# idra-lab/safe-mpc

Measured on AMD Instinct MI355X. Metric: RTI-MPC instance-steps/s (batch=4096 per GPU, Z1 N=30), higher is better.
Workload: dtype f64; 1 GPU; C1: Z1-class 6-DoF, N=30, 4096 instances/GPU, controller st (soft terminal NN row, MLP 12-256-256-256-1 fp32), EXT cost exact Hessian, 6 capsule pairs, Halton x0; batch_per_gpu=4096, batch_total=4096, horizon=30, controller=st, streams_per_gpu=3, qp_form=throughput, hip_graphs=False

## Files before the change

### safe_mpc_amd/csrc/engine.hip

```cpp
#include <hip/hip_runtime.h>

#include <cstdarg>
#include <cstdio>
#include <cstring>
#include <new>
#include <type_traits>
#include <vector>

#include "../../include/smpc.h"
#include "kernel_qp.hpp"
#include "kernel_qp_wg.hpp"
#include "kernel_build.hpp"
#include "kernels_callers.hpp"
#include "kernels_policy.hpp"
#include "kernels_mlp.hpp"
#include "kernels_nodes.hpp"
#include "kernels_sqp.hpp"
#include "kernels_guess.hpp"
#include "kernels_score.hpp"
#include "kernels_ik.hpp"
#include "kernels_rays.hpp"
#include "kernels_forecast.hpp"

using namespace smpc;
// ... 83 lines not shown
    DevBuf<double> d_nn;
    DevBuf<double> d_ws;
    int qp_mode = -2;
    DevBuf<double> d_hrec;
    bool wg_lds_raised[2] = {false, false};
    DevBuf<int32_t> d_order, d_last_it;
    int order_B = 0;
    DevBuf<int32_t> d_ord_hist;
    DevBuf<float> d_S, d_y, d_GS, d_dA, d_dB;
    DevBuf<int32_t> d_nn_idx;
    int32_t* d_nn_cnt = nullptr;
    DevBuf<float> d_act[SMPC_MAX_LAYERS];
    DevBuf<float> d_dg[SMPC_MAX_LAYERS];
    DevBuf<char> d_stage;
    ParamBlock chk{"check bounds"};
    ParamBlock gchk{"guess check bounds"};
    ParamBlock schk{"score bounds"};
    ParamBlock ikb{"inverse kinematics bounds"};
    DevBuf<char> d_roll;
    int timing = 0;
    int timed = 0;
    static constexpr int EV_RING = 64;
    hipEvent_t ev_sets[EV_RING][5] = {};
    bool ev_complete[EV_RING] = {};
    hipEvent_t* ev_t = ev_sets[0];
    int ev_cur = 0;
    bool timing_now = false;
    long timed_count = 0;
    std::vector<smpc_handle*> kids;
    hipEvent_t ev_fork = nullptr, ev_join = nullptr;
    DevBuf<unsigned long long> d_wstat;
    const uint8_t* d_active = nullptr;
    DevBuf<char> d_polw;
    float last_ms[4] = {0, 0, 0, 0};
    long mlp_rows_whole = 0;
    long mlp_rows_hint = 0;
    DevBuf<char> d_par;
    DevBuf<char> d_sqp;
    DevBuf<int32_t> d_guess;
    DevBuf<char> d_score;
    char err[256] = "";
};

namespace {

int fail(smpc_handle* h, int code, const char* fmt, ...) {
    char* dst = h ? h->err : g_create_err;
    va_list ap;
    va_start(ap, fmt);
    vsnprintf(dst, 256, fmt, ap);
    va_end(ap);
    return code;
}
#define HIPCHK(h, expr)                                                                                       \
    do {                                                                                                      \
        hipError_t e_ = (expr);                                                                               \
        if (e_ != hipSuccess) return fail(h, SMPC_EHIP, "%s failed: %s", #expr, hipGetErrorString(e_));        \
    } while (0)

bool capturing(const smpc_handle* h) {
    hipStreamCaptureStatus cs = hipStreamCaptureStatusNone;
    if (hipStreamIsCapturing(h->stream, &cs) != hipSuccess) { (void)hipGetLastError(); return false; }
    return cs != hipStreamCaptureStatusNone;
}

}
// ... 143 lines not shown
    HIPCHK(h, hipMemcpyAsync(h->d_lo.p, l.data(), l.size() * sizeof(double), hipMemcpyHostToDevice, h->stream));
    HIPCHK(h, hipMemcpyAsync(h->d_hi.p, u.data(), u.size() * sizeof(double), hipMemcpyHostToDevice, h->stream));
    HIPCHK(h, hipStreamSynchronize(h->stream));
    return SMPC_OK;
}

int ensure_mlp(smpc_handle* h, size_t M, int level = 2) {
    const size_t Mp = (M + 127) / 128 * 128, row = sizeof(float) * Mp, H = h->net->H;
    int rc;
    if ((rc = h->d_y.reserve(h, "network output", row))) return rc;
    for (int l = 0; level >= 1 && l + 1 < h->net->nlayers; l++)
        if ((rc = h->d_dg[l].reserve(h, "network activation derivatives", row * H))) return rc;
    if (level < 2) return SMPC_OK;
    if ((rc = h->d_S.reserve(h, "network features", row * MLP_KPAD)) || (rc = h->d_GS.reserve(h, "network gradients", row * MLP_NPAD)) ||
        (rc = h->d_dA.reserve(h, "network backward pass", row * H)) || (rc = h->d_dB.reserve(h, "network backward pass", row * H)))
        return rc;
    for (int l = 0; l + 1 < h->net->nlayers; l++)
        if ((rc = h->d_act[l].reserve(h, "network activations", row * H))) return rc;
    return SMPC_OK;
}

int ensure_nn_idx(smpc_handle* h, size_t M) {
    if (sizeof(int32_t) * (M + 1) <= h->d_nn_idx.cap) return SMPC_OK;
    const int rc = h->d_nn_idx.reserve(h, "network row list", sizeof(int32_t) * (M + 1));
    h->d_nn_cnt = h->d_nn_idx.cap ? h->d_nn_idx.p + h->d_nn_idx.cap / sizeof(int32_t) - 1 : nullptr;
    if (rc) return rc;
    HIPCHK(h, hipMemsetAsync(h->d_nn_cnt, 0, sizeof(int32_t), h->stream));
    return SMPC_OK;
}

CtxSrc rows_of_nodes(int per) { CtxSrc c; c.per = per; return c; }
CtxSrc rows_step_major(int B, long m0) { CtxSrc c; c.mod = B; c.m0 = (int)(m0 % B); c.j0 = (int)(m0 / B); return c; }

template <int NQ> int run_mlp(smpc_handle* h, int M, int mode, int N, const double* d_x, bool backward, CtxSrc rows,
                              const double* d_p = nullptr, double* d_ev = nullptr, bool* chained = nullptr, int compact = 0) {
    int rc;
    const Net& net = *h->net;
    CtxSrc cx = rows;
    if (net.n_ctx > 0) {
        const float* own = h->ctx.held();
        cx.n = net.n_ctx;
        cx.p = own ? own : net.d_default_ctx.p;
        cx.stride = own ? net.n_ctx : 0;
        cx.T = own ? (int)h->ctx_T : 1;
        cx.clock = cx.T > 1 && cx.mod == 0 && !(own && h->ctx_fc) ? h->scene_clock : nullptr;
    }
    const int Mp = (M + 127) / 128 * 128, H = net.H, L = net.nlayers;
    hipStream_t s = h->stream;
    const int32_t* idx = mode == 3 ? h->d_nn_idx.p : nullptr;
    const int32_t* live = mode == 3 ? h->d_nn_cnt : nullptr;
    if (chained) *chained = false;
    {
        const long rows_all = h->mlp_rows_whole > 0 ? (h->mlp_rows_whole + 127) / 128 * 128
                                                    : (h->mlp_rows_hint > 0 && mode == 3 ? (h->mlp_rows_hint + 127) / 128 * 128 : (long)Mp);
        static const bool no_fused = getenv("SMPC_MLP_UNFUSED") != nullptr;
        static const long fused_max = [] { const char* e = getenv("SMPC_MLP_FUSED_MAX"); return e ? atol(e) : 8192L; }();
        if (!no_fused && rows_all < fused_max && H == MLPF_H && L == 4 && (!backward || (d_p && d_ev))) {
            if ((rc = ensure_mlp(h, (size_t)M, 0))) return rc;
            MlpWeights Wt;
            for (int l = 0; l < SMPC_MAX_LAYERS; l++) { Wt.wf[l] = net.Wfwd[l]; Wt.wb[l] = net.Wbwd[l]; Wt.bias[l] = net.bias[l]; }
            const dim3 grd((M + MLPF_ROWS - 1) / MLPF_ROWS), blk(256);
            if (backward)
                hipLaunchKernelGGL((k_mlp_fused<NQ, true>), grd, blk, 0, s, h->d_desc, M, N, mode, net.act, Wt, d_x, d_p, idx, live, h->d_y.p, d_ev,
                                   compact, cx);
            else
                hipLaunchKernelGGL((k_mlp_fused<NQ, false>), grd, blk, 0, s, h->d_desc, M, N, mode, net.act, Wt, d_x, d_p, idx, live, h->d_y.p,
                                   (double*)nullptr, 0, cx);
            HIPCHK(h, hipGetLastError());
            if (chained) *chained = backward;
            return SMPC_OK;
        }
        static const bool large_chain = [] { const char* e = getenv("SMPC_MLP_LARGE"); return e && !strcmp(e, "chain"); }();
        if (!no_fused && !large_chain && rows_all >= fused_max && H == MLPF_H && L == 4 && (!backward || (d_p && d_ev))) {
            if ((rc = ensure_mlp(h, (size_t)M, backward ? 1 : 0))) return rc;
            MlpWeights Wt;
            for (int l = 0; l < SMPC_MAX_LAYERS; l++) { Wt.wf[l] = net.Wfwd[l]; Wt.wb[l] = net.Wbwd[l]; Wt.bias[l] = net.bias[l]; }
            const dim3 grd((M + MLPF_ROWS - 1) / MLPF_ROWS), blk(64);
            if (backward)
                hipLaunchKernelGGL((k_mlp_wave<NQ, true>), grd, blk, 0, s, h->d_desc, M, N, mode, net.act, Wt, d_x, d_p, idx, live, h->d_y.p, d_ev,
                                   compact, h->d_dg[0].p, h->d_dg[1].p, h->d_dg[2].p, cx);
            else
                hipLaunchKernelGGL((k_mlp_wave<NQ, false>), grd, blk, 0, s, h->d_desc, M, N, mode, net.act, Wt, d_x, d_p, idx, live, h->d_y.p,
                                   (double*)nullptr, 0, (float*)nullptr, (float*)nullptr, (float*)nullptr, cx);
            HIPCHK(h, hipGetLastError());
            if (chained) *chained = backward;
            return SMPC_OK;
        }
    }
    if ((rc = ensure_mlp(h, (size_t)M))) return rc;
    hipLaunchKernelGGL((k_nn_features<NQ>), dim3((Mp + 63) / 64), dim3(64), 0, s, h->d_desc, M, Mp, N, mode, d_x,
                       h->d_S.p, idx, live, cx);
    const dim3 blk(64), grd(Mp / 32, H / 64);
    hipLaunchKernelGGL((k_gemm_f32<EPI_BIAS_GELU>), grd, blk, 0, s, Mp, H, MLP_KPAD, h->d_S.p, net.Wfwd[0], net.bias[0],
                       (const float*)nullptr, h->d_act[0].p, h->d_dg[0].p, live, net.act);
    for (int l = 1; l + 1 < L; l++)
        hipLaunchKernelGGL((k_gemm_f32<EPI_BIAS_GELU>), grd, blk, 0, s, Mp, H, H, h->d_act[l - 1].p, net.Wfwd[l], net.bias[l],
                           (const float*)nullptr, h->d_act[l].p, h->d_dg[l].p, live, net.act);
    hipLaunchKernelGGL(k_nn_output, dim3((Mp + 3) / 4), dim3(256), 0, s, Mp, H, h->d_act[L - 2].p, h->d_dg[L - 2].p,
                       net.Wbwd[L - 1], net.bias[L - 1], h->d_y.p, h->d_dA.p, live);
    if (backward) {
        float *cur = h->d_dA.p, *nxt = h->d_dB.p;
        for (int l = L - 2; l >= 1; l--) {
            hipLaunchKernelGGL((k_gemm_f32<EPI_MUL>), grd, blk, 0, s, Mp, H, H, cur, net.Wbwd[l], (const float*)nullptr,
                               h->d_dg[l - 1].p, nxt, (float*)nullptr, live, net.act);
            float* t = cur; cur = nxt; nxt = t;
        }
        hipLaunchKernelGGL((k_gemm_f32<EPI_PLAIN>), dim3(Mp / 32, MLP_NPAD / 64), blk, 0, s, Mp, MLP_NPAD, H, cur,
                           net.Wbwd[0], (const float*)nullptr, (const float*)nullptr, h->d_GS.p, (float*)nullptr, live, net.act);
    }
    HIPCHK(h, hipGetLastError());
    return SMPC_OK;
}

template <int NQ>
int launch_nn(smpc_handle* h, int B, const double* d_xg, const double* d_p, double* d_out, int compact) {
    if (h->desc.nn_mode == SMPC_NN_NONE) return SMPC_OK;
    const int N = h->N;
    hipStream_t s = h->stream;
    if (h->net->nlayers == 0) return fail(h, SMPC_ESTATE, "nn_mode != NONE but smpc_set_mlp was not called");
    const int mode = h->desc.nn_mode == SMPC_NN_TERMINAL ? 1 : 3;
    const int M = mode == 1 ? B : B * N;
    int rc;
    if (mode == 3) {
        if ((rc = ensure_nn_idx(h, (size_t)M))) return rc;
        hipLaunchKernelGGL(k_nn_compact, dim3((M + 63) / 64), dim3(64), 0, s, M, N, d_p, h->d_nn_idx.p, h->d_nn_cnt);
    }
    bool chained = false;
    if ((rc = run_mlp<NQ>(h, M, mode, N, d_xg, true, rows_of_nodes(N + 1), d_p, d_out, &chained, compact))) return rc;
    if (!chained)
        hipLaunchKernelGGL((k_nn_chain<NQ>), dim3((M + 63) / 64), dim3(64), 0, s, h->d_desc, M, N, mode, d_xg, d_p,
                           h->d_y.p, h->d_GS.p, d_out, mode == 3 ? h->d_nn_idx.p : (const int32_t*)nullptr,
                           mode == 3 ? h->d_nn_cnt : (const int32_t*)nullptr, compact);
    HIPCHK(h, hipGetLastError());
    return SMPC_OK;
}

template <class F> int with_scene(const smpc_handle* h, int B, F&& f, int64_t off = 0, bool clocked = true) {
    if (const double* geom = h->scene.for_batch(B)) {
        if (h->scene_fc) return f(std::true_type{}, SceneSrc{geom, nullptr, h->scene_T, 0});
        return f(std::true_type{}, SceneSrc{geom, clocked && h->scene_T > 1 ? h->scene_clock : nullptr, h->scene_T, off});
    }
    return f(std::false_type{}, (const double*)nullptr);
}

template <class F> int with_model(const smpc_handle* h, int B, F&& f) {
    if (const ModelSrc table = h->models.for_batch(B)) return f(std::true_type{}, table);
    return f(std::false_type{});
}

int guard_scene_and_context(smpc_handle* h, int B, const char* who) {
    const int rc = h->scene.guard(h, B, who);
    return rc ? rc : h->ctx.guard(h, B, who);
}
int guard_scene_context_and_models(smpc_handle* h, int B, const char* who) {
    const int rc = guard_scene_and_context(h, B, who);
    return rc ? rc : h->models.guard(h, B, who);
}

void drop_forecast(smpc_handle* h) {
    if (h->scene_fc) h->scene.clear();
    if (h->ctx_fc) h->ctx.clear();
// ... 764 lines not shown

extern "C" {

int smpc_abi_version(void) { return SMPC_ABI_VERSION; }

const char* smpc_last_error(const smpc_handle* h) { return h ? h->err : g_create_err; }

int smpc_create(const smpc_problem_desc* desc, int device, smpc_handle** out) {
    if (!desc || !out) return fail(nullptr, SMPC_EINVAL, "null argument");
    *out = nullptr;
    if (stream_route() < 0)
        return fail(nullptr, SMPC_EINVAL, "SMPC_STREAM_PRIORITY=%s: expected default, high or low", getenv("SMPC_STREAM_PRIORITY"));
    if (desc->abi_version != SMPC_ABI_VERSION)
        return fail(nullptr, SMPC_EINVAL, "descriptor ABI %d, library ABI %d", desc->abi_version, SMPC_ABI_VERSION);
    if (desc->nq < 5 || desc->nq > SMPC_MAX_NQ) return fail(nullptr, SMPC_EINVAL, "nq=%d unsupported", desc->nq);
    if (desc->N < 1 || desc->N > SMPC_MAX_N) return fail(nullptr, SMPC_EINVAL, "N=%d outside 1..%d", desc->N, SMPC_MAX_N);
    if (desc->n_rows < 0 || desc->n_rows > SMPC_MAX_ROWS || desc->n_points < 1 || desc->n_points > SMPC_MAX_POINTS)
        return fail(nullptr, SMPC_EINVAL, "n_rows / n_points out of range");
    for (int i = 0; i < desc->n_points; i++)
        if (desc->points[i].link >= desc->nq) return fail(nullptr, SMPC_EINVAL, "point %d rides on link %d >= nq", i, desc->points[i].link);
    for (int r = 0; r < desc->n_rows; r++) {
        const smpc_row& row = desc->rows[r];
        if (row.kind < 0 || row.kind > SMPC_ROW_COORD || row.pa < 0 || row.pa >= desc->n_points)
            return fail(nullptr, SMPC_EINVAL, "row %d malformed", r);
    }
    if (3 * desc->nq + desc->n_rows + 1 > 32)
        return fail(nullptr, SMPC_EINVAL, "3*nq + n_rows + 1 = %d constraint rows per stage exceed the 32 lanes of a half-wavefront",
                    3 * desc->nq + desc->n_rows + 1);
    int ndev = 0;
    if (hipGetDeviceCount(&ndev) != hipSuccess || ndev <= 0)
        return fail(nullptr, SMPC_EHIP, "no HIP device visible: the engine has no CPU fallback");
    if (device < 0 || device >= ndev) return fail(nullptr, SMPC_EINVAL, "device %d of %d", device, ndev);
    smpc_handle* h = new (std::nothrow) smpc_handle();
    if (!h) return fail(nullptr, SMPC_ENOMEM, "out of host memory");
    h->desc = *desc;
    h->device = device;
    h->N = desc->N;
    hipError_t e = create_handle_stream(device, &h->stream);
    if (e == hipSuccess) e = hipMalloc((void**)&h->d_desc, sizeof(smpc_problem_desc));
    if (e == hipSuccess) e = hipMemcpy(h->d_desc, desc, sizeof(smpc_problem_desc), hipMemcpyHostToDevice);
    for (int i = 0; i < 5 * smpc_handle::EV_RING && e == hipSuccess; i++) e = hipEventCreate(&h->ev_sets[i / 5][i % 5]);
    if (e != hipSuccess) {
        fail(nullptr, SMPC_EHIP, "device setup failed: %s", hipGetErrorString(e));
        smpc_destroy(h);
        return SMPC_EHIP;
    }
    int rc = upload_bounds(h, nullptr, nullptr);
    if (rc) {
        snprintf(g_create_err, sizeof(g_create_err), "%s", h->err);
        smpc_destroy(h);
        return rc;
    }
    *out = h;
    return SMPC_OK;
}

void smpc_destroy(smpc_handle* h) {
    if (!h) return;
    (void)hipSetDevice(h->device);
    for (smpc_handle* k : h->kids) smpc_destroy(k);
    if (h->stream) (void)hipStreamSynchronize(h->stream);
    if (h->ev_fork) (void)hipEventDestroy(h->ev_fork);
    if (h->ev_join) (void)hipEventDestroy(h->ev_join);
    for (auto& set : h->ev_sets) for (auto& e : set) if (e) (void)hipEventDestroy(e);
    if (h->stream) (void)hipStreamDestroy(h->stream);
    if (h->d_desc) (void)hipFree(h->d_desc);
// ... 697 lines not shown
    if (B <= 0 || !par || !st || !x || !u_out || !abort_out || !any_abort) return fail(h, SMPC_EINVAL, "bad argument");
    if (!st->x_guess || !st->u_guess || !st->x_temp || !st->u_temp || !st->p || !st->x_viable || !st->fails ||
        !st->current_step || !st->status || !st->qp_iter)
        return fail(h, SMPC_EINVAL, "policy state incomplete");
    const int kind = par->kind;
    if (kind < SMPC_POLICY_NAIVE || kind > SMPC_POLICY_PARALLEL) return fail(h, SMPC_EINVAL, "unknown policy kind %d", kind);
    const bool receding = kind == SMPC_POLICY_RECEDING || kind == SMPC_POLICY_REAL_RECEDING;
    const bool parallel = kind == SMPC_POLICY_PARALLEL;
    if ((receding || parallel) && !st->r) return fail(h, SMPC_EINVAL, "receding policy without r");
    if (parallel && h->desc.nn_mode != SMPC_NN_ALL) return fail(h, SMPC_EINVAL, "parallel policy needs the safe-set row on every node (SMPC_NN_ALL)");
    if (kind == SMPC_POLICY_REAL_RECEDING && (!par->stage_lo || !par->stage_hi)) return fail(h, SMPC_EINVAL, "stage_lo / stage_hi missing");
    if (stepping && !u_other) return fail(h, SMPC_EINVAL, "u_other missing");
    if (kind != SMPC_POLICY_NAIVE && (!par->x_min || !par->x_max || (h->desc.n_rows > 0 && (!par->row_lb_chk || !par->row_ub_chk))))
        return fail(h, SMPC_EINVAL, "check bounds missing");
    if ((receding || parallel) && h->net->nlayers == 0) return fail(h, SMPC_ESTATE, "receding policy but smpc_set_mlp was not called");
    if (parallel)
        if (const int rf = refuse_slots(h, "smpc_policy_step", "the parallel policy's candidate slots are not instances",
                                            {&h->scene, &h->ctx, &h->models}))
            return rf;
    (void)hipSetDevice(h->device);
    const int N = h->N, nq = h->desc.nq, nx = 2 * nq;
    hipStream_t s = h->stream;
    int rc;
    if ((rc = guard_scene_context_and_models(h, B, "smpc_policy_step"))) return rc;
    TrajSrc tr;
    if (!parallel && (rc = policy_traj_src(h, B, st, &tr))) return rc;
    if ((rc = ensure_batch(h, B))) return rc;
    PolScratch w;
    if ((rc = policy_scratch(h, B, &w))) return rc;
    int32_t *d_ok = w.ok, *d_safe = w.safe, *d_acc = w.acc;
    uint8_t* d_act = w.act;
    if (kind != SMPC_POLICY_NAIVE && (rc = upload_check_bounds(h, par->x_min, par->x_max, par->row_lb_chk, par->row_ub_chk))) return rc;
    if (parallel) return policy_step_parallel(h, B, par, st, x, stepping, u_other, u_out, abort_out, any_abort, d_ok, d_safe, d_acc, d_act);
    if (kind != SMPC_POLICY_REAL_RECEDING)
        hipLaunchKernelGGL(k_guess_correction, dim3((B * nq + 63) / 64), dim3(64), 0, s, B, N, nq, h->desc.dt, st->x_guess,
                           st->u_guess, stepping, any_abort, d_ok);
    if (receding) {
        if (kind == SMPC_POLICY_REAL_RECEDING) {
            if ((rc = ensure_instance_bounds(h, B, true))) return rc;
            h->bounds.commit(B);
        }
        hipLaunchKernelGGL(k_policy_pre, dim3((unsigned)(((size_t)B * (N + 1) + 63) / 64)), dim3(64), 0, s, B, N, nx, kind,
                           stepping, st->r, st->p, st->x_guess, par->stage_lo, par->stage_hi, par->tube, h->bounds.d.p, instance_hi(h),
                           kind == SMPC_POLICY_REAL_RECEDING ? any_abort : (int32_t*)nullptr,
                           kind == SMPC_POLICY_REAL_RECEDING ? d_ok : (int32_t*)nullptr);
    }
    if (tr.p)
        hipLaunchKernelGGL(k_policy_traj, dim3((unsigned)(((size_t)B * (N + 1) + 63) / 64)), dim3(64), 0, s, B, N, stepping,
                           st->current_step, tr.p, tr.len, tr.stride, st->p);
    HIPCHK(h, hipGetLastError());
    h->d_active = stepping;
    h->mlp_rows_hint = receding ? 2L * B : 0L;
    rc = with_nq(h, [&](auto NQ) { return launch_solve<NQ>(h, B, x, st->x_guess, st->u_guess, st->p, st->x_temp, st->u_temp, st->status, st->qp_iter); });
    h->d_active = nullptr;
    if (rc) { h->mlp_rows_hint = 0; return rc; }
    if (kind != SMPC_POLICY_NAIVE) {
        const int coll = par->collision_first_node ? 1 : N + 1;
        if (receding) {
            const size_t M = (size_t)B * (N + 1);
            if ((rc = ensure_nn_idx(h, M))) return rc;
            hipLaunchKernelGGL(k_policy_safe_list, dim3((unsigned)((M + 63) / 64)), dim3(64), 0, s, B, N, par->abort_flag, stepping, st->r,
                               h->d_nn_idx.p, h->d_nn_cnt);
        }
        if ((rc = check_nodes_dev(h, B, N + 1, st->x_temp, par->tol_x, coll, par->alpha, par->tol_safe, d_ok, receding ? d_safe : nullptr,
                                  receding, true))) {
            h->mlp_rows_hint = 0;
            return rc;
        }
    }
    h->mlp_rows_hint = 0;
    hipLaunchKernelGGL(k_policy_post, dim3((B + 63) / 64), dim3(64), 0, s, B, N, nx, kind, par->abort_flag, stepping, st->status,
                       d_ok, d_safe, st->x_guess, st->fails, st->current_step, st->r, st->x_viable, d_acc, d_act, abort_out, any_abort,
                       (receding && kind != SMPC_POLICY_NAIVE) ? h->d_nn_cnt : (int32_t*)nullptr);

    hipLaunchKernelGGL(k_provide_control, dim3((B * (nx + nq) + 63) / 64), dim3(64), 0, s, B, N, nq, d_acc, st->x_temp, st->u_temp,
                       st->x_guess, st->u_guess, u_out, stepping, d_act, u_other);
    HIPCHK(h, hipGetLastError());
    return SMPC_OK;
}

int smpc_loop_pre(smpc_handle* h, int B, int Nb, const smpc_loop_state* ls, const int64_t* r, const uint8_t* pending, double* u_other,
                  uint8_t* stepping) {
    if (!h) return SMPC_EINVAL;
    if (B <= 0 || Nb <= 0 || !ls || !u_other || !stepping) return fail(h, SMPC_EINVAL, "bad argument");
    if (!ls->x_cur || !ls->alive || !ls->sa || !ls->ja || !ls->x_abort || !ls->u_abort || !ls->step)
        return fail(h, SMPC_EINVAL, "loop state incomplete");
    (void)hipSetDevice(h->device);
    hipLaunchKernelGGL(k_loop_pre, dim3((B + 63) / 64), dim3(64), 0, h->stream, B, h->desc.nq, Nb, ls->x_cur, ls->alive, ls->sa,
// ... 444 lines not shown
    int rc;
    if ((rc = guard_scene_context_and_models(h, B, "smpc_debug_stage_records"))) return rc;
    if ((rc = ensure_batch(h, B))) return rc;
    const int N = h->N, nx = 2 * h->desc.nq, nu = h->desc.nq;
    Stage io{h, false};
    const double *dx0, *dxg, *dug, *dp;
    if ((rc = io.place([&](Stage& v) {
             dx0 = v.in(x0, (size_t)B * nx);
             dxg = v.in(xg, (size_t)B * (N + 1) * nx);
             dug = v.in(ug, (size_t)B * N * nu);
             dp = v.in(p, (size_t)B * (N + 1) * SMPC_NP);
         })))
        return rc;
    const size_t per = ws_doubles_per_instance(h, N);
    HIPCHK(h, hipMemsetAsync(h->d_ws.p, 0, per * (size_t)B * sizeof(double), h->stream));
    (void)&launch_stage_records<5>, (void)&launch_stage_records_per_node<5>;
    (void)&launch_stage_records<6>, (void)&launch_stage_records_per_node<6>;
    (void)&launch_stage_records<7>, (void)&launch_stage_records_per_node<7>;
    if ((rc = with_nq(h, [&](auto NQ) {
             return path == 1 ? launch_stage_records<NQ>(h, B, dx0, dxg, dug, dp, false) : launch_stage_records_per_node<NQ>(h, B, dx0, dxg, dug, dp);
         })))
        return rc;
    HIPCHK(h, hipMemcpyAsync(ws_out, h->d_ws.p, per * (size_t)B * sizeof(double), hipMemcpyDeviceToHost, h->stream));
    if ((rc = io.finish())) return rc;
    return with_nq(h, [&](auto NQ) {
        const QpLayout<NQ> Ly(h->desc.n_rows);
        const int v[24] = {Ly.stride, Ly.nIMG, Ly.oIMG, Ly.oSL, Ly.nF, Ly.oR0, Ly.oR1, Ly.oR2, Ly.oCZA, Ly.oCZN, Ly.oZ, Ly.oZN, Ly.NRT, Ly.nJ,
                           (int)per, 12, Ly.iTT, Ly.iGT, Ly.iGN, Ly.iB, Ly.iSC, Ly.iHQQ, Ly.iGZ, 0};
        for (int i = 0; i < 24; i++) layout[i] = v[i];
        return SMPC_OK;
    });
}

#ifdef QP_PROFILE
extern "C" int smpc_debug_qp_profile(unsigned long long* out16) {
    unsigned long long zero[16] = {0};
    if (hipMemcpyFromSymbol(out16, HIP_SYMBOL(smpc::g_qp_prof), sizeof(zero)) != hipSuccess) return -1;
    if (hipMemcpyToSymbol(HIP_SYMBOL(smpc::g_qp_prof), zero, sizeof(zero)) != hipSuccess) return -1;
    return 0;
}
extern "C" int smpc_debug_qp_wg_profile(unsigned long long* out16) {
    unsigned long long zero[16] = {0};
    if (hipMemcpyFromSymbol(out16, HIP_SYMBOL(smpc::g_wg_prof), sizeof(zero)) != hipSuccess) return -1;
    if (hipMemcpyToSymbol(HIP_SYMBOL(smpc::g_wg_prof), zero, sizeof(zero)) != hipSuccess) return -1;
    return 0;
}
#endif
```

### safe_mpc_amd/csrc/kernels_callers.hpp

```cpp
#pragma once
#include "device_model.hpp"

namespace smpc {

__global__ void k_guess_correction(int B, int N, int nq, double dt, double* __restrict__ xg,
                                   const double* __restrict__ ug, const uint8_t* __restrict__ mask, int32_t* __restrict__ zero_flag,
                                   int32_t* __restrict__ ok_fill) {
    const long t = (long)blockIdx.x * blockDim.x + threadIdx.x;
    if (t == 0 && zero_flag) *zero_flag = 0;
    if (t >= (long)B * nq) return;
    const long b = t / nq;
    const int i = (int)(t % nq);
    if (ok_fill && i == 0) ok_fill[b] = 1;
    if (mask && !mask[b]) return;
    const int nx = 2 * nq;
    double* x = xg + b * (N + 1) * nx;
    const double* u = ug + b * N * nq;
    double q = x[i], v = x[nq + i];
    const double c = 0.5 * dt * dt;
    for (int k = 0; k < N; k++) {
        const double uk = u[k * nq + i];
        q = q + dt * v + c * uk;
        v = v + dt * uk;
        x[(k + 1) * nx + i] = q;
        x[(k + 1) * nx + nq + i] = v;
    }
}

__global__ void k_provide_control(int B, int N, int nq, const int32_t* __restrict__ accept,
                                  const double* __restrict__ xt, const double* __restrict__ ut,
                                  double* __restrict__ xg, double* __restrict__ ug, double* __restrict__ u_apply,
                                  const uint8_t* __restrict__ stepping, const uint8_t* __restrict__ active,
                                  const double* __restrict__ u_other) {
    const int nx = 2 * nq, ncol = nx + nq;
    const long t = (long)blockIdx.x * blockDim.x + threadIdx.x;
    if (t >= (long)B * ncol) return;
    const long b = t / ncol;
    const int c = (int)(t % ncol);
    const bool acc = accept[b] != 0;
    const bool stp = !stepping || stepping[b], act = stp && (!active || active[b]);
    if (!act) {
        if (c >= nx) u_apply[b * nq + c - nx] = stp ? ug[b * N * nq + c - nx] : u_other[b * nq + c - nx];
        return;
    }
    if (c < nx) {
        double* x = xg + b * (N + 1) * nx;
        const double* src = acc ? xt + b * (N + 1) * nx : x;
        for (int k = 0; k < N; k++) x[k * nx + c] = src[(k + 1) * nx + c];
        x[N * nx + c] = x[(N - 1) * nx + c];
    } else {
        const int i = c - nx;
        double* u = ug + b * N * nq;
        const double* src = acc ? ut + b * N * nq : u;
        u_apply[b * nq + i] = src[i];
        for (int k = 0; k + 1 < N; k++) u[k * nq + i] = src[(k + 1) * nq + i];
        if (N > 1) u[(N - 1) * nq + i] = u[(N - 2) * nq + i];
        else u[i] = src[i];
    }
}

template <int NQ>
__device__ __forceinline__ bool node_box_ok(const double* __restrict__ xk, const double* __restrict__ x_min, const double* __restrict__ x_max,
                                            double tol_x) {
    constexpr int NX = 2 * NQ;
    bool ok = true;
#pragma unroll
    for (int i = 0; i < NX; i++) ok = ok && (xk[i] >= x_min[i] - tol_x) && (xk[i] <= x_max[i] + tol_x);
    return ok;
}
template <int NQ, bool SCENE>
__device__ __forceinline__ bool node_rows_ok(const smpc_problem_desc* __restrict__ D, const double* __restrict__ xk, bool ok,
                                             const double* __restrict__ row_lb, const double* __restrict__ row_ub,
                                             const double* __restrict__ geom_b) {
    double q[NQ];
#pragma unroll
    for (int i = 0; i < NQ; i++) q[i] = xk[i];
    Mat3<double> Rw[NQ];
    Vec3<double> pw[NQ], zw[NQ];
    fk_world<NQ>(D->joints, q, Rw, pw, zw);
    for (int r = 0; r < D->n_rows; r++) {
        const smpc_row& row = D->rows[r];
        const double v = row_value<0, SCENE>(row, row_geom<SCENE>(row, geom_b, r), [&](int i) { return point_world(D->points[i], Rw, pw); }).v;
        ok = ok && (row_lb[r] <= v) && (v <= row_ub[r]);
    }
    return ok;
}

template <int NQ, bool SCENE = false>
__global__ void k_check_nodes(const smpc_problem_desc* __restrict__ D, int B, int n_nodes, const double* __restrict__ x,
                              const double* __restrict__ x_min, const double* __restrict__ x_max, double tol_x,
                              const double* __restrict__ row_lb, const double* __restrict__ row_ub,
// ... 149 lines not shown
```

### safe_mpc_amd/csrc/kernels_mlp.hpp

```cpp
#pragma once
#include <hip/hip_runtime.h>

#include <type_traits>

#include "device_model.hpp"

namespace smpc {

typedef float f32x16 __attribute__((ext_vector_type(16)));
typedef float f32x4 __attribute__((ext_vector_type(4)));

constexpr int MLP_KPAD = 16;
constexpr int MLP_NPAD = 64;

__device__ __forceinline__ float gelu_tanh_f(float a, float* dg) {
    const float k0 = 0.7978845608028654f, k1 = 0.044715f;
    const float a2 = a * a;
    const float inner = k0 * (a + k1 * a * a2);
    const float th = tanhf(inner);
    *dg = 0.5f * (1.0f + th) + 0.5f * a * (1.0f - th * th) * k0 * (1.0f + 3.0f * k1 * a2);
    return 0.5f * a * (1.0f + th);
}

__device__ __forceinline__ float act_f(int act, float a, float* dg) {
    switch (act) {
    case SMPC_ACT_RELU: *dg = a > 0.0f ? 1.0f : 0.0f; return a > 0.0f ? a : 0.0f;
    case SMPC_ACT_ELU: { const float e = expf(a); *dg = a > 0.0f ? 1.0f : e; return a > 0.0f ? a : e - 1.0f; }
    case SMPC_ACT_TANH: { const float t = tanhf(a); *dg = 1.0f - t * t; return t; }
    case SMPC_ACT_SILU: { const float sg = 1.0f / (1.0f + expf(-a)); *dg = sg * (1.0f + a * (1.0f - sg)); return a * sg; }
    default: return gelu_tanh_f(a, dg);
    }
}

enum { EPI_BIAS_GELU = 0, EPI_MUL = 1, EPI_PLAIN = 2 };

template <int EPI>
__global__ __launch_bounds__(256) void k_gemm_f32(int M, int N, int K, const float* __restrict__ A,
                                                  const float* __restrict__ Bm, const float* __restrict__ bias,
// ... 184 lines not shown
    const float* gs = GS + (size_t)m * MLP_NPAD;
    double v[NQ], vn2 = 0.0, gdv = 0.0;
#pragma unroll
    for (int i = 0; i < NQ; i++) {
        v[i] = i < nd ? x[NQ + i] + (i == 0 ? D->nn_eps : 0.0) : 0.0;
        vn2 += v[i] * v[i];
    }
    const double vn = sqrt(vn2);
#pragma unroll
    for (int i = 0; i < NQ; i++)
        if (i < nd) gdv += (double)gs[nd + i] * v[i];
    const double kap = (100.0 - pk[3]) / 100.0;
    o[o_val * es] = (double)y[m] * kap - vn;
#pragma unroll
    for (int i = 0; i < NQ; i++) {
        if (i < nd) {
            o[(o_grad + i) * es] = kap * (double)gs[i] / D->nn_std[i];
            o[(o_grad + NQ + i) * es] = kap * ((double)gs[nd + i] / vn - v[i] * gdv / (vn * vn * vn)) - v[i] / vn;
        }
    }
}

struct MlpWeights {
    const float* wf[SMPC_MAX_LAYERS];
    const float* wb[SMPC_MAX_LAYERS];
    const float* bias[SMPC_MAX_LAYERS];
};
constexpr int MLPF_ROWS = 16, MLPF_H = 256, MLPF_LD = MLPF_H + 4;

template <int NQ, bool BWD>
__global__ __launch_bounds__(256) void k_mlp_fused(const smpc_problem_desc* __restrict__ D, int M, int N, int mode, int act,
                                                   MlpWeights Wt, const double* __restrict__ xg, const double* __restrict__ p,
                                                   const int32_t* __restrict__ idx, const int32_t* __restrict__ m_live,
                                                   float* __restrict__ y_out, double* __restrict__ ev_out, int compact, CtxSrc cx) {
    constexpr int H = MLPF_H, LD = MLPF_LD, R = MLPF_ROWS;
    __shared__ __attribute__((aligned(16))) float bufA[R * LD];
    __shared__ __attribute__((aligned(16))) float bufB[R * LD];
    __shared__ __attribute__((aligned(16))) float sfeat[R * MLP_KPAD];
    __shared__ float sy[R];
    __shared__ float sgs[4 * R * 16];
    const int t = threadIdx.x, w = t >> 6, lane = t & 63, j = lane & 15, kq = lane >> 4;
    const int m0 = blockIdx.x * R;
    const int live = m_live ? *m_live : M;
    if (m0 >= live) return;
    if (t < R) nn_feature_row<NQ>(D, xg, mode, N, m0 + t, m0 + t < live, idx, cx, sfeat + t * MLP_KPAD);
    __syncthreads();
    const int c0 = 64 * w + 4 * j;
    f32x4 acc[4];
    float dg[3][4][4];
    auto zero_acc = [&]() {
#pragma unroll
        for (int tt = 0; tt < 4; tt++) acc[tt] = f32x4{0.0f, 0.0f, 0.0f, 0.0f};
    };
    auto chunk = [&](const f32x4 av, const f32x4* bv) {
#pragma unroll
        for (int r = 0; r < 4; r++) {
#pragma unroll
            for (int tt = 0; tt < 4; tt++) acc[tt] = __builtin_amdgcn_mfma_f32_16x16x4f32(av[r], bv[r][tt], acc[tt], 0, 0, 0);
        }
    };
    auto gemm = [&](const float* In, int ld_in, const float* __restrict__ Bm, int K) {
        const float* arow = In + j * ld_in + 4 * kq;
        const float* brow = Bm + (size_t)(4 * kq) * H + c0;
        f32x4 bq[4][4];
        auto bload = [&](f32x4* bv, int c) {
#pragma unroll
            for (int r = 0; r < 4; r++) bv[r] = *reinterpret_cast<const f32x4*>(brow + (size_t)(16 * c + r) * H);
        };
        bload(bq[0], 0);
        if (K == 16) {
            chunk(*reinterpret_cast<const f32x4*>(arow), bq[0]);
            return;
        }
        const int nch = K >> 4;
        bload(bq[1], 1);
        bload(bq[2], 2);
        bload(bq[3], 3);
// ... 326 lines not shown
```

### safe_mpc_amd/csrc/kernels_policy.hpp

```cpp
#pragma once
#include "device_model.hpp"
#include "kernels_callers.hpp"

namespace smpc {

__global__ void k_policy_pre(int B, int N, int nx, int kind, const uint8_t* __restrict__ stepping,
                             const int64_t* __restrict__ r_all, double* __restrict__ p, const double* __restrict__ xg,
                             const double* __restrict__ lo_st, const double* __restrict__ hi_st, double tube,
                             double* __restrict__ lo_b, double* __restrict__ hi_b, int32_t* __restrict__ zero_flag,
                             int32_t* __restrict__ ok_fill) {
    const long t = (long)blockIdx.x * blockDim.x + threadIdx.x;
    if (t == 0 && zero_flag) *zero_flag = 0;
    if (t >= (long)B * (N + 1)) return;
    const long b = t / (N + 1);
    const int k = (int)(t - b * (N + 1));
    if (ok_fill && k == 0) ok_fill[b] = 1;
    if (stepping && !stepping[b]) return;
    const int r = (int)r_all[b];
    if (kind == SMPC_POLICY_RECEDING) {
        const bool on = k == N || (k == r && r < N) || k == 0;
        p[t * SMPC_NP + 4] = on ? 1.0 : -1.0;
    } else {
        const bool at_r = k == r && r < N;
        const int rc = (r < N - 1 ? r : N - 1) + 1;
// ... 5 lines not shown
    }
}

__global__ void k_policy_traj(int B, int N, const uint8_t* __restrict__ stepping, const int64_t* __restrict__ current_step,
                              const double* __restrict__ traj, long traj_len, long stride, double* __restrict__ p) {
    const long t = (long)blockIdx.x * blockDim.x + threadIdx.x;
    if (t >= (long)B * (N + 1)) return;
    const long b = t / (N + 1);
    const int k = (int)(t - b * (N + 1));
    if (stepping && !stepping[b]) return;
    long c = (long)current_step[b] + k;
    c = c < 0 ? 0 : (c < traj_len ? c : traj_len - 1);
    const double* tb = traj + (size_t)b * stride;
    for (int i = 0; i < 3; i++) p[t * SMPC_NP + i] = tb[(size_t)i * traj_len + c];
}

__global__ void k_policy_safe_list(int B, int N, int abort_flag, const uint8_t* __restrict__ stepping, const int64_t* __restrict__ r_all,
                                   int32_t* __restrict__ idx, int32_t* __restrict__ count) {
    const long t = (long)blockIdx.x * blockDim.x + threadIdx.x;
    if (t >= (long)B * (N + 1)) return;
    const long b = t / (N + 1);
    const int k = (int)(t - b * (N + 1));
    if (stepping && !stepping[b]) return;
    int64_t r = r_all[b];
    if (abort_flag) {
        r -= 1;
        if (r == 0) r += N;
    } else {
        r -= r > 0 ? 1 : 0;
    }
    if (k >= r + 2) idx[atomicAdd(count, 1)] = (int32_t)t;
}

__global__ void k_policy_post(int B, int N, int nx, int kind, int abort_flag, const uint8_t* __restrict__ stepping,
                              const int32_t* __restrict__ status, const int32_t* __restrict__ state_ok,
                              const int32_t* __restrict__ safe, const double* __restrict__ xg, int64_t* __restrict__ fails,
                              int64_t* __restrict__ current_step, int64_t* __restrict__ r_all, double* __restrict__ x_viable,
                              int32_t* __restrict__ accept, uint8_t* __restrict__ active, uint8_t* __restrict__ abort_out,
                              int32_t* __restrict__ any_abort, int32_t* __restrict__ zero_cnt) {
    const int b = blockIdx.x * blockDim.x + threadIdx.x;
    if (b == 0 && zero_cnt) *zero_cnt = 0;
    if (b >= B) return;
    if (stepping && !stepping[b]) {
        accept[b] = 0;
        active[b] = 0;
        abort_out[b] = 0;
        return;
    }
    const double* xgb = xg + (size_t)b * (N + 1) * nx;
    int64_t f = fails[b];
    bool abort = false;
    if (kind == SMPC_POLICY_NAIVE || kind == SMPC_POLICY_STATE_CHECK) {
        const bool ok = status[b] == 0 && (kind == SMPC_POLICY_NAIVE || state_ok[b] != 0);
        f = ok ? 0 : f + 1;
    } else if (kind == SMPC_POLICY_STWA) {
        const bool ok = status[b] == 0 && state_ok[b] != 0;
        if (!ok && f == 0)
            for (int i = 0; i < nx; i++) x_viable[(size_t)b * nx + i] = xgb[(size_t)(N - 1) * nx + i];
        abort = !ok && f == N - 1;
        f = ok ? 0 : (abort ? f : f + 1);
    } else {
        int64_t r = r_all[b];
        if (abort_flag) {
            r -= 1;
            abort = r == 0;
        } else {
            r -= r > 0 ? 1 : 0;
        }
        if (abort) {
            for (int i = 0; i < nx; i++) x_viable[(size_t)b * nx + i] = xgb[(size_t)nx + i];
            r += N;
        }
        const bool ok = status[b] == 0 && state_ok[b] != 0 && !abort;
        int best = -1;
        for (int i = (int)r + 2; i <= N; i++)
            if (safe[(size_t)b * (N + 1) + i]) best = i;
        if (ok && best >= 0) r = best - 1;
        r_all[b] = r;
        f = abort ? f : (ok ? 0 : f + 1);
    }
    fails[b] = f;
    current_step[b] += abort ? 0 : 1;
    accept[b] = f == 0;
    active[b] = !abort;
    abort_out[b] = abort;
    if (abort) atomicOr(any_abort, 1);
}


__device__ __forceinline__ double par_flag(int k, int n, double own0) { return k == 0 ? own0 : (k == n ? 1.0 : -1.0); }

__device__ __forceinline__ int par_result(int n, int N, int r, int status, int state_ok, const int32_t* __restrict__ safe) {
    if (status != 0 || !state_ok) return 0;
    int checked = 0;
    for (int i = r > 0 ? r : 0; i <= N; i++)
        if (safe[i]) checked = i;
    const int cv = checked >= r ? checked : (n < r ? n : r);
    return cv >= r ? cv : 0;
}

__global__ void k_par_fanout1(int B, int N, const uint8_t* __restrict__ stepping, const double* __restrict__ p,
                              double* __restrict__ p1, int32_t* __restrict__ n_open) {
    const long t = (long)blockIdx.x * blockDim.x + threadIdx.x;
    if (t == 0) *n_open = 0;
    if (t >= (long)B * (N + 1)) return;
    const long b = t / (N + 1);
    const int k = (int)(t - b * (N + 1));
    const double* src = p + t * SMPC_NP;
    double* dst = p1 + t * SMPC_NP;
    for (int i = 0; i < 4; i++) dst[i] = src[i];
    const bool stp = !stepping || stepping[b];
    dst[4] = stp ? par_flag(k, N, p[b * (N + 1) * SMPC_NP + 4]) : (k == 0 ? src[4] : -1.0);
}

__global__ void k_par_safe_list(int S, int N, int K, const uint8_t* __restrict__ stepping, const int32_t* __restrict__ list,
                                const int32_t* __restrict__ n_open, const int64_t* __restrict__ r_all, const int32_t* __restrict__ status,
                                int32_t* __restrict__ idx, int32_t* __restrict__ count) {
    const long t = (long)blockIdx.x * blockDim.x + threadIdx.x;
    if (t >= (long)S * (N + 1)) return;
// ... 242 lines not shown
```

Baseline: 1.149 million instance-steps/s.

## Fuse guess correction into MLP kernel and policy checks into single tail kernel

For the non-receding policy step, the separate guess-correction kernel is deferred and folded into the fused terminal MLP kernel, which applies the correction per block before building features. The post-solve state check, policy bookkeeping and provide-control kernels are merged into one k_policy_tail kernel that handles two instances per 64-thread block, using half-wave shuffles to reduce the check result and broadcast the accept/active flags. This aims to cut kernel launches and global round trips per step. The cost is extra work inside the MLP kernel and some coupling between the solver path and policy state. An environment switch restores the old path.

```diff
diff --git a/safe_mpc_amd/csrc/engine.hip b/safe_mpc_amd/csrc/engine.hip
--- a/safe_mpc_amd/csrc/engine.hip
+++ b/safe_mpc_amd/csrc/engine.hip
@@ -139,6 +139,8 @@
     DevBuf<unsigned long long> d_wstat;
     const uint8_t* d_active = nullptr;
     DevBuf<char> d_polw;
+    bool policy_fused = true;
+    GuessFix pending_fix;
     float last_ms[4] = {0, 0, 0, 0};
     long mlp_rows_whole = 0;
     long mlp_rows_hint = 0;
@@ -348,8 +350,22 @@
 CtxSrc rows_of_nodes(int per) { CtxSrc c; c.per = per; return c; }
 CtxSrc rows_step_major(int B, long m0) { CtxSrc c; c.mod = B; c.m0 = (int)(m0 % B); c.j0 = (int)(m0 / B); return c; }
 
+int mlp_route(const smpc_handle* h, int M, int mode, bool backward, bool chain_args) {
+    const Net& net = *h->net;
+    const long Mp = (M + 127) / 128 * 128;
+    const long rows_all = h->mlp_rows_whole > 0 ? (h->mlp_rows_whole + 127) / 128 * 128
+                                                : (h->mlp_rows_hint > 0 && mode == 3 ? (h->mlp_rows_hint + 127) / 128 * 128 : Mp);
+    static const bool no_fused = getenv("SMPC_MLP_UNFUSED") != nullptr;
+    static const long fused_max = [] { const char* e = getenv("SMPC_MLP_FUSED_MAX"); return e ? atol(e) : 8192L; }();
+    static const bool large_chain = [] { const char* e = getenv("SMPC_MLP_LARGE"); return e && !strcmp(e, "chain"); }();
+    if (no_fused || net.H != MLPF_H || net.nlayers != 4 || (backward && !chain_args)) return 0;
+    if (rows_all < fused_max) return 1;
+    return large_chain ? 0 : 2;
+}
+
 template <int NQ> int run_mlp(smpc_handle* h, int M, int mode, int N, const double* d_x, bool backward, CtxSrc rows,
-                              const double* d_p = nullptr, double* d_ev = nullptr, bool* chained = nullptr, int compact = 0) {
+                              const double* d_p = nullptr, double* d_ev = nullptr, bool* chained = nullptr, int compact = 0,
+                              const GuessFix& fix = {}) {
     int rc;
     const Net& net = *h->net;
     CtxSrc cx = rows;
@@ -367,27 +383,23 @@
     const int32_t* live = mode == 3 ? h->d_nn_cnt : nullptr;
     if (chained) *chained = false;
     {
-        const long rows_all = h->mlp_rows_whole > 0 ? (h->mlp_rows_whole + 127) / 128 * 128
-                                                    : (h->mlp_rows_hint > 0 && mode == 3 ? (h->mlp_rows_hint + 127) / 128 * 128 : (long)Mp);
-        static const bool no_fused = getenv("SMPC_MLP_UNFUSED") != nullptr;
-        static const long fused_max = [] { const char* e = getenv("SMPC_MLP_FUSED_MAX"); return e ? atol(e) : 8192L; }();
-        if (!no_fused && rows_all < fused_max && H == MLPF_H && L == 4 && (!backward || (d_p && d_ev))) {
+        const int route = mlp_route(h, M, mode, backward, d_p && d_ev);
+        if (route == 1) {
             if ((rc = ensure_mlp(h, (size_t)M, 0))) return rc;
             MlpWeights Wt;
             for (int l = 0; l < SMPC_MAX_LAYERS; l++) { Wt.wf[l] = net.Wfwd[l]; Wt.wb[l] = net.Wbwd[l]; Wt.bias[l] = net.bias[l]; }
             const dim3 grd((M + MLPF_ROWS - 1) / MLPF_ROWS), blk(256);
             if (backward)
                 hipLaunchKernelGGL((k_mlp_fused<NQ, true>), grd, blk, 0, s, h->d_desc, M, N, mode, net.act, Wt, d_x, d_p, idx, live, h->d_y.p, d_ev,
-                                   compact, cx);
+                                   compact, cx, fix);
             else
                 hipLaunchKernelGGL((k_mlp_fused<NQ, false>), grd, blk, 0, s, h->d_desc, M, N, mode, net.act, Wt, d_x, d_p, idx, live, h->d_y.p,
-                                   (double*)nullptr, 0, cx);
+                                   (double*)nullptr, 0, cx, GuessFix{});
             HIPCHK(h, hipGetLastError());
             if (chained) *chained = backward;
             return SMPC_OK;
         }
-        static const bool large_chain = [] { const char* e = getenv("SMPC_MLP_LARGE"); return e && !strcmp(e, "chain"); }();
-        if (!no_fused && !large_chain && rows_all >= fused_max && H == MLPF_H && L == 4 && (!backward || (d_p && d_ev))) {
+        if (route == 2) {
             if ((rc = ensure_mlp(h, (size_t)M, backward ? 1 : 0))) return rc;
             MlpWeights Wt;
             for (int l = 0; l < SMPC_MAX_LAYERS; l++) { Wt.wf[l] = net.Wfwd[l]; Wt.wb[l] = net.Wbwd[l]; Wt.bias[l] = net.bias[l]; }
@@ -430,9 +442,16 @@
 
 template <int NQ>
 int launch_nn(smpc_handle* h, int B, const double* d_xg, const double* d_p, double* d_out, int compact) {
-    if (h->desc.nn_mode == SMPC_NN_NONE) return SMPC_OK;
     const int N = h->N;
     hipStream_t s = h->stream;
+    GuessFix fix = h->pending_fix;
+    h->pending_fix = GuessFix{};
+    if (fix.xg && !(h->desc.nn_mode == SMPC_NN_TERMINAL && h->net->nlayers != 0 && mlp_route(h, B, 1, true, d_p && d_out) == 1)) {
+        hipLaunchKernelGGL(k_guess_correction, dim3((B * fix.nq + 63) / 64), dim3(64), 0, s, B, N, fix.nq, fix.dt, fix.xg, fix.ug, fix.mask,
+                           fix.zero_flag, fix.ok_fill);
+        fix = GuessFix{};
+    }
+    if (h->desc.nn_mode == SMPC_NN_NONE) return SMPC_OK;
     if (h->net->nlayers == 0) return fail(h, SMPC_ESTATE, "nn_mode != NONE but smpc_set_mlp was not called");
     const int mode = h->desc.nn_mode == SMPC_NN_TERMINAL ? 1 : 3;
     const int M = mode == 1 ? B : B * N;
@@ -442,7 +461,7 @@
         hipLaunchKernelGGL(k_nn_compact, dim3((M + 63) / 64), dim3(64), 0, s, M, N, d_p, h->d_nn_idx.p, h->d_nn_cnt);
     }
     bool chained = false;
-    if ((rc = run_mlp<NQ>(h, M, mode, N, d_xg, true, rows_of_nodes(N + 1), d_p, d_out, &chained, compact))) return rc;
+    if ((rc = run_mlp<NQ>(h, M, mode, N, d_xg, true, rows_of_nodes(N + 1), d_p, d_out, &chained, compact, fix))) return rc;
     if (!chained)
         hipLaunchKernelGGL((k_nn_chain<NQ>), dim3((M + 63) / 64), dim3(64), 0, s, h->d_desc, M, N, mode, d_xg, d_p,
                            h->d_y.p, h->d_GS.p, d_out, mode == 3 ? h->d_nn_idx.p : (const int32_t*)nullptr,
@@ -1273,6 +1292,10 @@
         return fail(nullptr, SMPC_EHIP, "no HIP device visible: the engine has no CPU fallback");
     if (device < 0 || device >= ndev) return fail(nullptr, SMPC_EINVAL, "device %d of %d", device, ndev);
     smpc_handle* h = new (std::nothrow) smpc_handle();
+    if (h) {
+        const char* e = getenv("SMPC_POLICY_FUSED");
+        h->policy_fused = !e || atoi(e) != 0;
+    }
     if (!h) return fail(nullptr, SMPC_ENOMEM, "out of host memory");
     h->desc = *desc;
     h->device = device;
@@ -2036,7 +2059,8 @@
     uint8_t* d_act = w.act;
     if (kind != SMPC_POLICY_NAIVE && (rc = upload_check_bounds(h, par->x_min, par->x_max, par->row_lb_chk, par->row_ub_chk))) return rc;
     if (parallel) return policy_step_parallel(h, B, par, st, x, stepping, u_other, u_out, abort_out, any_abort, d_ok, d_safe, d_acc, d_act);
-    if (kind != SMPC_POLICY_REAL_RECEDING)
+    const bool fused = h->policy_fused && !receding;
+    if (!fused && kind != SMPC_POLICY_REAL_RECEDING)
         hipLaunchKernelGGL(k_guess_correction, dim3((B * nq + 63) / 64), dim3(64), 0, s, B, N, nq, h->desc.dt, st->x_guess,
                            st->u_guess, stepping, any_abort, d_ok);
     if (receding) {
@@ -2054,10 +2078,31 @@
                            st->current_step, tr.p, tr.len, tr.stride, st->p);
     HIPCHK(h, hipGetLastError());
     h->d_active = stepping;
+    if (fused) h->pending_fix = GuessFix{st->x_guess, st->u_guess, stepping, any_abort, nullptr, h->desc.dt, nq};
     h->mlp_rows_hint = receding ? 2L * B : 0L;
     rc = with_nq(h, [&](auto NQ) { return launch_solve<NQ>(h, B, x, st->x_guess, st->u_guess, st->p, st->x_temp, st->u_temp, st->status, st->qp_iter); });
     h->d_active = nullptr;
+    h->pending_fix = GuessFix{};
     if (rc) { h->mlp_rows_hint = 0; return rc; }
+    if (fused) {
+        h->mlp_rows_hint = 0;
+        const ChkBlock c = chk_block(h->chk.d.p, nq);
+        const int coll = par->collision_first_node ? 1 : N + 1;
+        const dim3 grd((unsigned)((B + 1) / 2)), blk(64);
+        const auto launch = [&](auto NQ, auto SCENE, auto CHECK, auto sc) {
+            hipLaunchKernelGGL((k_policy_tail<NQ, SCENE, CHECK>), grd, blk, 0, s, h->d_desc, B, N, kind, par->abort_flag, stepping, st->status,
+                               st->x_temp, st->u_temp, c.x_min, c.x_max, par->tol_x, c.row_lb, c.row_ub, coll, st->x_guess, st->u_guess,
+                               st->fails, st->current_step, st->x_viable, d_acc, d_act, abort_out, any_abort, u_out, u_other, sc);
+            return SMPC_OK;
+        };
+        rc = with_nq(h, [&](auto NQ) {
+            if (kind == SMPC_POLICY_NAIVE) return launch(NQ, std::false_type{}, std::false_type{}, (const double*)nullptr);
+            return with_scene(h, B, [&](auto SCENE, auto sc) { return launch(NQ, SCENE, std::true_type{}, sc); });
+        });
+        if (rc) return rc;
+        HIPCHK(h, hipGetLastError());
+        return SMPC_OK;
+    }
     if (kind != SMPC_POLICY_NAIVE) {
         const int coll = par->collision_first_node ? 1 : N + 1;
         if (receding) {
@@ -2568,6 +2613,15 @@
     });
 }
 
+extern "C" int smpc_debug_order(smpc_handle* h, int B, int32_t* out) {
+    if (!h || B <= 0 || !out) return SMPC_EINVAL;
+    (void)hipSetDevice(h->device);
+    if (h->order_B != B || h->d_order.cap < sizeof(int32_t) * (size_t)B) return fail(h, SMPC_ESTATE, "no dispatch order for %d instances", B);
+    HIPCHK(h, hipMemcpyAsync(out, h->d_order.p, sizeof(int32_t) * (size_t)B, hipMemcpyDeviceToHost, h->stream));
+    HIPCHK(h, hipStreamSynchronize(h->stream));
+    return SMPC_OK;
+}
+
 #ifdef QP_PROFILE
 extern "C" int smpc_debug_qp_profile(unsigned long long* out16) {
     unsigned long long zero[16] = {0};
diff --git a/safe_mpc_amd/csrc/kernels_callers.hpp b/safe_mpc_amd/csrc/kernels_callers.hpp
--- a/safe_mpc_amd/csrc/kernels_callers.hpp
+++ b/safe_mpc_amd/csrc/kernels_callers.hpp
@@ -3,14 +3,19 @@
 
 namespace smpc {
 
-__global__ void k_guess_correction(int B, int N, int nq, double dt, double* __restrict__ xg,
-                                   const double* __restrict__ ug, const uint8_t* __restrict__ mask, int32_t* __restrict__ zero_flag,
-                                   int32_t* __restrict__ ok_fill) {
-    const long t = (long)blockIdx.x * blockDim.x + threadIdx.x;
-    if (t == 0 && zero_flag) *zero_flag = 0;
-    if (t >= (long)B * nq) return;
-    const long b = t / nq;
-    const int i = (int)(t % nq);
+struct GuessFix {
+    double* xg = nullptr;
+    const double* ug = nullptr;
+    const uint8_t* mask = nullptr;
+    int32_t* zero_flag = nullptr;
+    int32_t* ok_fill = nullptr;
+    double dt = 0.0;
+    int nq = 0;
+};
+
+__device__ __forceinline__ void guess_correction_joint(long b, int i, int N, int nq, double dt, double* __restrict__ xg,
+                                                       const double* __restrict__ ug, const uint8_t* __restrict__ mask,
+                                                       int32_t* __restrict__ ok_fill) {
     if (ok_fill && i == 0) ok_fill[b] = 1;
     if (mask && !mask[b]) return;
     const int nx = 2 * nq;
@@ -27,18 +32,20 @@
     }
 }
 
-__global__ void k_provide_control(int B, int N, int nq, const int32_t* __restrict__ accept,
-                                  const double* __restrict__ xt, const double* __restrict__ ut,
-                                  double* __restrict__ xg, double* __restrict__ ug, double* __restrict__ u_apply,
-                                  const uint8_t* __restrict__ stepping, const uint8_t* __restrict__ active,
-                                  const double* __restrict__ u_other) {
-    const int nx = 2 * nq, ncol = nx + nq;
-    const long t = (long)blockIdx.x * blockDim.x + threadIdx.x;
-    if (t >= (long)B * ncol) return;
-    const long b = t / ncol;
-    const int c = (int)(t % ncol);
-    const bool acc = accept[b] != 0;
-    const bool stp = !stepping || stepping[b], act = stp && (!active || active[b]);
+__global__ void k_guess_correction(int B, int N, int nq, double dt, double* __restrict__ xg,
+                                   const double* __restrict__ ug, const uint8_t* __restrict__ mask, int32_t* __restrict__ zero_flag,
+                                   int32_t* __restrict__ ok_fill) {
+    const long t = (long)blockIdx.x * blockDim.x + threadIdx.x;
+    if (t == 0 && zero_flag) *zero_flag = 0;
+    if (t >= (long)B * nq) return;
+    guess_correction_joint(t / nq, (int)(t % nq), N, nq, dt, xg, ug, mask, ok_fill);
+}
+
+__device__ __forceinline__ void provide_control_column(long b, int c, int N, int nq, bool acc, bool stp, bool act,
+                                                       const double* __restrict__ xt, const double* __restrict__ ut,
+                                                       double* __restrict__ xg, double* __restrict__ ug, double* __restrict__ u_apply,
+                                                       const double* __restrict__ u_other) {
+    const int nx = 2 * nq;
     if (!act) {
         if (c >= nx) u_apply[b * nq + c - nx] = stp ? ug[b * N * nq + c - nx] : u_other[b * nq + c - nx];
         return;
@@ -57,6 +64,21 @@
         if (N > 1) u[(N - 1) * nq + i] = u[(N - 2) * nq + i];
         else u[i] = src[i];
     }
+}
+
+__global__ void k_provide_control(int B, int N, int nq, const int32_t* __restrict__ accept,
+                                  const double* __restrict__ xt, const double* __restrict__ ut,
+                                  double* __restrict__ xg, double* __restrict__ ug, double* __restrict__ u_apply,
+                                  const uint8_t* __restrict__ stepping, const uint8_t* __restrict__ active,
+                                  const double* __restrict__ u_other) {
+    const int ncol = 3 * nq;
+    const long t = (long)blockIdx.x * blockDim.x + threadIdx.x;
+    if (t >= (long)B * ncol) return;
+    const long b = t / ncol;
+    const int c = (int)(t % ncol);
+    const bool acc = accept[b] != 0;
+    const bool stp = !stepping || stepping[b], act = stp && (!active || active[b]);
+    provide_control_column(b, c, N, nq, acc, stp, act, xt, ut, xg, ug, u_apply, u_other);
 }
 
 template <int NQ>
diff --git a/safe_mpc_amd/csrc/kernels_mlp.hpp b/safe_mpc_amd/csrc/kernels_mlp.hpp
--- a/safe_mpc_amd/csrc/kernels_mlp.hpp
+++ b/safe_mpc_amd/csrc/kernels_mlp.hpp
@@ -4,6 +4,7 @@
 #include <type_traits>
 
 #include "device_model.hpp"
+#include "kernels_callers.hpp"
 
 namespace smpc {
 
@@ -254,7 +255,8 @@
 __global__ __launch_bounds__(256) void k_mlp_fused(const smpc_problem_desc* __restrict__ D, int M, int N, int mode, int act,
                                                    MlpWeights Wt, const double* __restrict__ xg, const double* __restrict__ p,
                                                    const int32_t* __restrict__ idx, const int32_t* __restrict__ m_live,
-                                                   float* __restrict__ y_out, double* __restrict__ ev_out, int compact, CtxSrc cx) {
+                                                   float* __restrict__ y_out, double* __restrict__ ev_out, int compact, CtxSrc cx,
+                                                   GuessFix gf = {}) {
     constexpr int H = MLPF_H, LD = MLPF_LD, R = MLPF_ROWS;
     __shared__ __attribute__((aligned(16))) float bufA[R * LD];
     __shared__ __attribute__((aligned(16))) float bufB[R * LD];
@@ -265,6 +267,12 @@
     const int m0 = blockIdx.x * R;
     const int live = m_live ? *m_live : M;
     if (m0 >= live) return;
+    if (gf.xg) {
+        if (blockIdx.x == 0 && t == 0 && gf.zero_flag) *gf.zero_flag = 0;
+        if (t < R * gf.nq && m0 + t / gf.nq < M) guess_correction_joint(m0 + t / gf.nq, t % gf.nq, N, gf.nq, gf.dt, gf.xg, gf.ug, gf.mask, gf.ok_fill);
+        __syncthreads();
+        xg = gf.xg;
+    }
     if (t < R) nn_feature_row<NQ>(D, xg, mode, N, m0 + t, m0 + t < live, idx, cx, sfeat + t * MLP_KPAD);
     __syncthreads();
     const int c0 = 64 * w + 4 * j;
diff --git a/safe_mpc_amd/csrc/kernels_policy.hpp b/safe_mpc_amd/csrc/kernels_policy.hpp
--- a/safe_mpc_amd/csrc/kernels_policy.hpp
+++ b/safe_mpc_amd/csrc/kernels_policy.hpp
@@ -61,29 +61,26 @@
     if (k >= r + 2) idx[atomicAdd(count, 1)] = (int32_t)t;
 }
 
-__global__ void k_policy_post(int B, int N, int nx, int kind, int abort_flag, const uint8_t* __restrict__ stepping,
-                              const int32_t* __restrict__ status, const int32_t* __restrict__ state_ok,
-                              const int32_t* __restrict__ safe, const double* __restrict__ xg, int64_t* __restrict__ fails,
-                              int64_t* __restrict__ current_step, int64_t* __restrict__ r_all, double* __restrict__ x_viable,
-                              int32_t* __restrict__ accept, uint8_t* __restrict__ active, uint8_t* __restrict__ abort_out,
-                              int32_t* __restrict__ any_abort, int32_t* __restrict__ zero_cnt) {
-    const int b = blockIdx.x * blockDim.x + threadIdx.x;
-    if (b == 0 && zero_cnt) *zero_cnt = 0;
-    if (b >= B) return;
+__device__ __forceinline__ int policy_post_instance(int b, int N, int nx, int kind, int abort_flag, const uint8_t* __restrict__ stepping,
+                                                    const int32_t* __restrict__ status, bool state_ok, const int32_t* __restrict__ safe,
+                                                    const double* xg, int64_t* __restrict__ fails, int64_t* __restrict__ current_step,
+                                                    int64_t* __restrict__ r_all, double* __restrict__ x_viable,
+                                                    int32_t* __restrict__ accept, uint8_t* __restrict__ active,
+                                                    uint8_t* __restrict__ abort_out, int32_t* __restrict__ any_abort) {
     if (stepping && !stepping[b]) {
         accept[b] = 0;
         active[b] = 0;
         abort_out[b] = 0;
-        return;
+        return 0;
     }
     const double* xgb = xg + (size_t)b * (N + 1) * nx;
     int64_t f = fails[b];
     bool abort = false;
     if (kind == SMPC_POLICY_NAIVE || kind == SMPC_POLICY_STATE_CHECK) {
-        const bool ok = status[b] == 0 && (kind == SMPC_POLICY_NAIVE || state_ok[b] != 0);
+        const bool ok = status[b] == 0 && (kind == SMPC_POLICY_NAIVE || state_ok);
         f = ok ? 0 : f + 1;
     } else if (kind == SMPC_POLICY_STWA) {
-        const bool ok = status[b] == 0 && state_ok[b] != 0;
+        const bool ok = status[b] == 0 && state_ok;
         if (!ok && f == 0)
             for (int i = 0; i < nx; i++) x_viable[(size_t)b * nx + i] = xgb[(size_t)(N - 1) * nx + i];
         abort = !ok && f == N - 1;
@@ -100,7 +97,7 @@
             for (int i = 0; i < nx; i++) x_viable[(size_t)b * nx + i] = xgb[(size_t)nx + i];
             r += N;
         }
-        const bool ok = status[b] == 0 && state_ok[b] != 0 && !abort;
+        const bool ok = status[b] == 0 && state_ok && !abort;
         int best = -1;
         for (int i = (int)r + 2; i <= N; i++)
             if (safe[(size_t)b * (N + 1) + i]) best = i;
@@ -114,6 +111,67 @@
     active[b] = !abort;
     abort_out[b] = abort;
     if (abort) atomicOr(any_abort, 1);
+    return (f == 0 ? 1 : 0) | (abort ? 0 : 2);
+}
+
+__global__ void k_policy_post(int B, int N, int nx, int kind, int abort_flag, const uint8_t* __restrict__ stepping,
+                              const int32_t* __restrict__ status, const int32_t* __restrict__ state_ok,
+                              const int32_t* __restrict__ safe, const double* __restrict__ xg, int64_t* __restrict__ fails,
+                              int64_t* __restrict__ current_step, int64_t* __restrict__ r_all, double* __restrict__ x_viable,
+                              int32_t* __restrict__ accept, uint8_t* __restrict__ active, uint8_t* __restrict__ abort_out,
+                              int32_t* __restrict__ any_abort, int32_t* __restrict__ zero_cnt) {
+    const int b = blockIdx.x * blockDim.x + threadIdx.x;
+    if (b == 0 && zero_cnt) *zero_cnt = 0;
+    if (b >= B) return;
+    policy_post_instance(b, N, nx, kind, abort_flag, stepping, status, kind == SMPC_POLICY_NAIVE || state_ok[b] != 0, safe, xg, fails,
+                         current_step, r_all, x_viable, accept, active, abort_out, any_abort);
+}
+
+template <int NQ, bool SCENE, bool CHECK>
+__global__ __launch_bounds__(64) void k_policy_tail(const smpc_problem_desc* __restrict__ D, int B, int N, int kind, int abort_flag,
+                                                    const uint8_t* __restrict__ stepping, const int32_t* __restrict__ status,
+                                                    const double* xt, const double* __restrict__ ut, const double* __restrict__ x_min,
+                                                    const double* __restrict__ x_max, double tol_x, const double* __restrict__ row_lb,
+                                                    const double* __restrict__ row_ub, int coll_nodes, double* xg,
+                                                    double* __restrict__ ug, int64_t* __restrict__ fails,
+                                                    int64_t* __restrict__ current_step, double* __restrict__ x_viable,
+                                                    int32_t* __restrict__ accept, uint8_t* __restrict__ active,
+                                                    uint8_t* __restrict__ abort_out, int32_t* __restrict__ any_abort,
+                                                    double* __restrict__ u_apply, const double* __restrict__ u_other,
+                                                    const SceneArg<SCENE> sc = {}) {
+    constexpr int NX = 2 * NQ, HALF = 32;
+    static_assert(NX + NQ <= HALF, "provideControl's columns must fit a half-wavefront");
+    const int l = threadIdx.x & (HALF - 1);
+    const long b = (long)blockIdx.x * 2 + (threadIdx.x >> 5);
+    const bool live = b < B;
+    int ok = 1;
+    if constexpr (CHECK) {
+        if (live) {
+            bool okl = true;
+            for (int k = l; k <= N; k += HALF) {
+                const double* xk = xt + (b * (N + 1) + k) * NX;
+                bool okk = node_box_ok<NQ>(xk, x_min, x_max, tol_x);
+                if (k < coll_nodes) {
+                    const double* geom_b = nullptr;
+                    if constexpr (SCENE) geom_b = scene_block(sc, b, scene_time(sc) + k, D->n_rows);
+                    okk = node_rows_ok<NQ, SCENE>(D, xk, okk, row_lb, row_ub, geom_b);
+                }
+                okl = okl && okk;
+            }
+            ok = okl;
+        }
+        for (int o = HALF / 2; o > 0; o >>= 1) ok &= __shfl_xor(ok, o);
+    }
+    int flags = 0;
+    if (live && l == 0)
+        flags = policy_post_instance((int)b, N, NX, kind, abort_flag, stepping, status, ok != 0, nullptr, xg, fails, current_step, nullptr,
+                                     x_viable, accept, active, abort_out, any_abort);
+    __builtin_amdgcn_fence(__ATOMIC_ACQ_REL, "wavefront");
+    __builtin_amdgcn_wave_barrier();
+    flags = __shfl(flags, threadIdx.x & HALF);
+    if (!live || l >= NX + NQ) return;
+    const bool stp = !stepping || stepping[b];
+    provide_control_column(b, l, N, NQ, (flags & 1) != 0, stp, stp && (flags & 2) != 0, xt, ut, xg, ug, u_apply, u_other);
 }
 
 
```

Result: no change. 1.141 million instance-steps/s (-0.7%).
